# QizhiPei/FABind

Hardware: AMD Instinct MI355X
Metric: complexes/sec fwd+bwd (1500p/40l nodes), full IaBNet on the whole graph (pocket model + 4-layer complex model + distance-map head on all nodes / pairs) with the pocket-cls + pocket-centre + coord + distmap + distmap-by-coords + distill losses (BASELINE configs[2] read literally) (higher is better)
Workload: dtype bf16

## Files before the change

### fabind_amd/csrc/fused_common.h

```cpp
#pragma once
#include "common.h"

#define FE_BM 64
#define FE_PRIO(x) __builtin_amdgcn_s_setprio(x)

__device__ __forceinline__ float fe_sigmoid(float x) { return __builtin_amdgcn_rcpf(1.0f + __builtin_amdgcn_exp2f(-1.44269504f * x)); }
__device__ __forceinline__ float fe_silu(float x) { return x * fe_sigmoid(x); }

__device__ __forceinline__ uint32_t fe_hash(uint32_t x) {
    x ^= x >> 16; x *= 0x7feb352dU; x ^= x >> 15; x *= 0x846ca68bU; x ^= x >> 16;
    return x;
}
__device__ __forceinline__ float fe_keep(uint32_t seed, uint32_t e, uint32_t c, uint32_t H, uint32_t thr16, float scale) {
    const uint32_t h = fe_hash(seed + (e >> 1) * H + c);
    return (((e & 1u) ? (h >> 16) : (h & 0xffffu)) >= thr16) ? scale : 0.f;
}

__device__ __forceinline__ void unpack8(const uint4 u, float* f) {
    f[0] = __uint_as_float(u.x << 16); f[1] = __uint_as_float(u.x & 0xffff0000u);
    f[2] = __uint_as_float(u.y << 16); f[3] = __uint_as_float(u.y & 0xffff0000u);
    f[4] = __uint_as_float(u.z << 16); f[5] = __uint_as_float(u.z & 0xffff0000u);
    f[6] = __uint_as_float(u.w << 16); f[7] = __uint_as_float(u.w & 0xffff0000u);
}
__device__ __forceinline__ uint4 pack8(const float* f) {
// ... 268 lines not shown
        }
    }
    if (ne > 0) {
        if (first && head_cont) bnd_tile[c] = run;
        else if (tail_cont) bnd_tile[H + c] = run;
        else put(cur, run);
    }
    return pwr;
}

template <int H, bool WITH_RH, int SWZ>
__device__ __forceinline__ float fe_scan_runs64(const bf16_t* sX, const int* sRow, const float* sRh, int ne, bool head_cont,
                                                bool tail_cont, float* out, unsigned ld, float* bnd_tile, int c,
                                                bf16_t* out16 = nullptr, unsigned ld16 = 0, const bf16_t* sXlo = nullptr) {
    const int lane = threadIdx.x & 63;
    const int mine = sRow[lane], prev = sRow[max(lane - 1, 0)];
    const float rhl = WITH_RH ? sRh[lane] : 0.f;
    const unsigned long long m = __ballot(lane < ne && lane > 0 && mine != prev);
    const int c8 = c >> 3, c7 = c & 7;
    float v[64];
#pragma unroll
    for (int rw = 0; rw < 64; ++rw) v[rw] = bf16_to_f32(sX[rw * H + ((c8 ^ (rw & SWZ)) * 8) + c7]);
    if (sXlo) {
#pragma unroll
        for (int rw = 0; rw < 64; ++rw) v[rw] += bf16_to_f32(sXlo[rw * H + ((c8 ^ (rw & SWZ)) * 8) + c7]);
    }
    float run = 0.f, pwr = 0.f;
    int rs = 0;
    auto flush = [&](bool last) {
        if (rs == 0 && head_cont) bnd_tile[c] = run;
        else if (last && tail_cont) bnd_tile[H + c] = run;
        else {
            const unsigned node = (unsigned)__builtin_amdgcn_readlane(mine, rs);
            if (out) out[node * ld + c] = run;
            if (out16) out16[node * ld16 + c] = f32_to_bf16(run);
        }
    };
#pragma unroll
    for (int rw = 0; rw < 64; ++rw) {
        if (rw < ne) {
            if ((m >> rw) & 1ull) {
                flush(false);
                run = 0.f;
                rs = rw;
            }
            run += v[rw];
            if (WITH_RH) pwr += __builtin_bit_cast(float, __builtin_amdgcn_readlane(__builtin_bit_cast(int, rhl), rw)) * v[rw];
        }
    }
    if (ne > 0) flush(true);
    return pwr;
}

template <int BM>
__global__ void fe_boundary_fix_kernel(const int* __restrict__ row, int E, int H, const float* __restrict__ bnd, float* out,
                                       unsigned ld, bf16_t* out16 = nullptr, unsigned ld16 = 0) {
    const int t = blockIdx.x, e0 = t * BM, ne = min(BM, E - e0);
    if (ne <= 0 || e0 + ne >= E) return;
    const int r = row[e0 + ne - 1];
    if (row[e0 + ne] != r) return;
    if (row[e0] == r && e0 > 0 && row[e0 - 1] == r) return;
    for (int c = threadIdx.x; c < H; c += blockDim.x) {
        float sum = bnd[((size_t)t * 2 + 1) * H + c];
        for (int u = t + 1;; ++u) {
            const int f0 = u * BM, fn = min(BM, E - f0);
            sum += bnd[((size_t)u * 2) * H + c];
            const bool through = row[f0 + fn - 1] == r && f0 + fn < E && row[f0 + fn] == r;
            if (!through) break;
        }
        if (out) out[(unsigned)r * ld + c] = sum;
        if (out16) out16[(unsigned)r * ld16 + c] = f32_to_bf16(sum);
    }
}

__device__ __forceinline__ float fe3_row16_sum(float v) {
#define FE_DPP_ADD(ctrl_) v += __builtin_bit_cast(float, __builtin_amdgcn_update_dpp(0, __builtin_bit_cast(int, v), (ctrl_), 0xF, 0xF, true))
    FE_DPP_ADD(0xB1);
    FE_DPP_ADD(0x4E);
    FE_DPP_ADD(0x141);
    FE_DPP_ADD(0x140);
#undef FE_DPP_ADD
    return v;
}

typedef float fe_f2 __attribute__((ext_vector_type(2)));
__device__ __forceinline__ void fe3_silu_pair(const fe_f2 z, fe_f2& m, fe_f2& d) {
    const fe_f2 t = z * -1.44269504f;
    const fe_f2 o = fe_f2{__builtin_amdgcn_exp2f(t.x), __builtin_amdgcn_exp2f(t.y)} + 1.0f;
    const fe_f2 s = fe_f2{__builtin_amdgcn_rcpf(o.x), __builtin_amdgcn_rcpf(o.y)};
    m = z * s;
    d = s + (m - m * s);
}
__device__ __forceinline__ uint32_t fe3_pack(const fe_f2 v) { return pack2_bf16(v.x, v.y); }
__device__ __forceinline__ fe_f2 fe3_unpack(const uint32_t u) { return fe_f2{__uint_as_float(u << 16), __uint_as_float(u & 0xffff0000u)}; }

__device__ __forceinline__ uint4 fe3_bload16(const __amdgpu_buffer_rsrc_t rs, const unsigned voff, const unsigned soff) {
    const fe_u32x4_t v = __builtin_amdgcn_raw_buffer_load_b128(rs, (int)voff, (int)soff, 0);
    return make_uint4(v.x, v.y, v.z, v.w);
}
__device__ __forceinline__ void fe3_bstore16(const __amdgpu_buffer_rsrc_t rs, const unsigned voff, const unsigned soff, const uint4 v) {
    __builtin_amdgcn_raw_buffer_store_b128(fe_u32x4_t{v.x, v.y, v.z, v.w}, rs, (int)voff, (int)soff, 0);
}

struct FabindEdgeBwdArgs;
int fe_bwd3_launch(const FabindEdgeBwdArgs* a, int H, int bm, int n_groups, hipStream_t stream);
int fe_fwd3_launch(const float* AB, int ldab, int H, const int* row, const int* col, const float* rhohat, const float* w_r,
                   const void* W2ph, const void* W2pl, const float* b2, const void* Wcph, const void* Wcpl, const float* bc,
                   const float* w3, int E, float* agg, float* s_out, uint32_t thr16, float dscale, unsigned seed, float* bnd,
                   int xcd_aware, hipStream_t stream, void* Msave = nullptr, void* d2f = nullptr, void* z3f = nullptr);
int fe_fwd2_launch(const void* AB, int ldab, int H, const int* row, const int* col, const float* rhohat, const float* w_r,
                   const void* W2p, const float* b2, const void* Wcp, const float* bc, const float* w3, int E, float* agg,
                   float* s_out, uint32_t thr16, float dscale, unsigned seed, float* bnd, void* agg16, int xcd_aware, hipStream_t stream,
                   void* Msave = nullptr, void* d2f = nullptr, void* z3f = nullptr);
int fe_bwd4_launch(const FabindEdgeBwdArgs* a, int H, int n_groups, hipStream_t stream);
```

### fabind_amd/csrc/fused_edge.hip

```cpp
#include "common.h"
#include "fabind_hip.h"
#include "fused_common.h"

static int g_fe_xcd_aware = 1;
extern "C" void fabind_gcl_edge_fused_set_xcd_aware(int on) { g_fe_xcd_aware = on ? 1 : 0; }
static int g_fe_fwd_variant = 1;
extern "C" int fabind_gcl_edge_fused_set_variant(int v) {
    FB_REQUIRE(v == 1, "fabind_gcl_edge_fused_set_variant: 1 (row-wise / operand-swapped) is the only forward form built (variant 0 was retired in round 5)");
    g_fe_fwd_variant = v;
    return 0;
}
extern "C" int fabind_gcl_edge_fused_variant(void) { return g_fe_fwd_variant; }

static int fe_fwd_entry(const void* AB, int ldab, int H, const int* row, const int* col, const float* rhohat,
                        const float* w_r, const void* W2p, const float* b2, const void* Wcp, const float* bc,
                        const float* w3, int E, float* agg, float* s_out, float p_drop, unsigned seed,
                        float* bnd, void* agg16, void* Msave, void* d2f, void* z3f, hipStream_t stream) {
    if (E <= 0) return 0;
    FB_REQUIRE((Msave != nullptr) == (d2f != nullptr) && (Msave != nullptr) == (z3f != nullptr),
               "fabind_gcl_edge_fused_train: M, d2f and z3f come together");
    FB_REQUIRE(Msave == nullptr || g_fe_fwd_variant == 1, "fabind_gcl_edge_fused_train: the saving forward is the row-wise / operand-swapped kernel (variant 1)");
    FB_REQUIRE(bnd != nullptr, "fabind_gcl_edge_fused: bnd (ceil(E/64) x 2 x H floats of scratch) is required");
    FB_REQUIRE(p_drop >= 0.f && p_drop < 1.f, "fabind_gcl_edge_fused: p_drop in [0, 1)");
    const uint32_t thr16 = (uint32_t)(p_drop * 65536.0f + 0.5f);
    const float dscale = 1.0f / (1.0f - (float)thr16 / 65536.0f);
    FB_REQUIRE(H == 512 || H == 256 || H == 128 || H == 64, "fabind_gcl_edge_fused: H must be 64, 128, 256 or 512");
    FB_REQUIRE(ldab % 8 == 0, "fabind_gcl_edge_fused: ldab % 8");
    {
        const int rc = fe_fwd2_launch(AB, ldab, H, row, col, rhohat, w_r, W2p, b2, Wcp, bc, w3, E, agg, s_out, thr16, dscale, seed, bnd,
                                      agg16, g_fe_xcd_aware, stream, Msave, d2f, z3f);
        if (rc) return rc;
    }
    hipLaunchKernelGGL((fe_boundary_fix_kernel<FE_BM>), dim3((E + FE_BM - 1) / FE_BM), dim3(H < 256 ? H : 256), 0, stream, row, E, H,
                       bnd, agg, (unsigned)H, (bf16_t*)agg16, (unsigned)H);
    FB_CHECK_LAUNCH();
    return 0;
}

extern "C" int fabind_gcl_edge_fused(const void* AB, int ldab, int H, const int* row, const int* col, const float* rhohat,
                                     const float* w_r, const void* W2p, const float* b2, const void* Wcp, const float* bc,
                                     const float* w3, int E, float* agg, float* s_out, float p_drop, unsigned seed,
                                     float* bnd, void* agg16, hipStream_t stream) {
    return fe_fwd_entry(AB, ldab, H, row, col, rhohat, w_r, W2p, b2, Wcp, bc, w3, E, agg, s_out, p_drop, seed, bnd, agg16, nullptr, nullptr,
                        nullptr, stream);
}
extern "C" int fabind_gcl_edge_fused_train(const void* AB, int ldab, int H, const int* row, const int* col, const float* rhohat,
                                           const float* w_r, const void* W2p, const float* b2, const void* Wcp, const float* bc,
                                           const float* w3, int E, float* agg, float* s_out, float p_drop, unsigned seed,
                                           float* bnd, void* agg16, void* M, void* d2f, void* z3f, hipStream_t stream) {
    FB_REQUIRE(M != nullptr && d2f != nullptr && z3f != nullptr, "fabind_gcl_edge_fused_train: M, d2f, z3f are required");
    return fe_fwd_entry(AB, ldab, H, row, col, rhohat, w_r, W2p, b2, Wcp, bc, w3, E, agg, s_out, p_drop, seed, bnd, agg16, M, d2f, z3f, stream);
}

static int fe_x3_entry(const float* AB, int ldab, int n_rows, int H, const int* row, const int* col, const float* rhohat,
                       const float* w_r, const void* W2ph, const void* W2pl, const float* b2, const void* Wcph,
                       const void* Wcpl, const float* bc, const float* w3, int E, float* agg, float* s_out,
                       float p_drop, unsigned seed, float* bnd, void* Msave, void* d2f, void* z3f, hipStream_t stream) {
    if (E <= 0) return 0;
    FB_REQUIRE(bnd != nullptr, "fabind_gcl_edge_fused_x3: bnd (ceil(E/64) x 2 x H floats of scratch) is required");
    FB_REQUIRE(p_drop >= 0.f && p_drop < 1.f, "fabind_gcl_edge_fused_x3: p_drop in [0, 1)");
    FB_REQUIRE(H == 512 || H == 256 || H == 128 || H == 64, "fabind_gcl_edge_fused_x3: H must be 64, 128, 256 or 512");
    FB_REQUIRE(ldab % 4 == 0 && ((uintptr_t)AB & 15) == 0, "fabind_gcl_edge_fused_x3: AB must be 16-byte aligned with ldab % 4 == 0");
    FB_REQUIRE(n_rows >= 0 && (size_t)n_rows * (size_t)ldab * 4 < ((size_t)1 << 32), "fabind_gcl_edge_fused_x3: AB larger than 4 GiB (n_rows * ldab * 4 bytes): split the batch");
    const uint32_t thr16 = (uint32_t)(p_drop * 65536.0f + 0.5f);
    const float dscale = 1.0f / (1.0f - (float)thr16 / 65536.0f);
    const int rc = fe_fwd3_launch(AB, ldab, H, row, col, rhohat, w_r, W2ph, W2pl, b2, Wcph, Wcpl, bc, w3, E, agg, s_out, thr16, dscale,
                                  seed, bnd, g_fe_xcd_aware, stream, Msave, d2f, z3f);
    if (rc) return rc;
    hipLaunchKernelGGL((fe_boundary_fix_kernel<FE_BM>), dim3((E + FE_BM - 1) / FE_BM), dim3(H < 256 ? H : 256), 0, stream, row, E, H,
                       bnd, agg, (unsigned)H, (bf16_t*)nullptr, 0u);
    FB_CHECK_LAUNCH();
    return 0;
}
extern "C" int fabind_gcl_edge_fused_x3(const float* AB, int ldab, int n_rows, int H, const int* row, const int* col, const float* rhohat,
                                        const float* w_r, const void* W2ph, const void* W2pl, const float* b2, const void* Wcph,
                                        const void* Wcpl, const float* bc, const float* w3, int E, float* agg, float* s_out,
                                        float p_drop, unsigned seed, float* bnd, hipStream_t stream) {
    return fe_x3_entry(AB, ldab, n_rows, H, row, col, rhohat, w_r, W2ph, W2pl, b2, Wcph, Wcpl, bc, w3, E, agg, s_out, p_drop, seed, bnd,
                       nullptr, nullptr, nullptr, stream);
}
extern "C" int fabind_gcl_edge_fused_x3_train(const float* AB, int ldab, int n_rows, int H, const int* row, const int* col, const float* rhohat,
                                              const float* w_r, const void* W2ph, const void* W2pl, const float* b2, const void* Wcph,
                                              const void* Wcpl, const float* bc, const float* w3, int E, float* agg, float* s_out,
                                              float p_drop, unsigned seed, float* bnd, void* M, void* d2f, void* z3f, hipStream_t stream) {
    FB_REQUIRE(M != nullptr && d2f != nullptr && z3f != nullptr, "fabind_gcl_edge_fused_x3_train: M, d2f, z3f are required");
    return fe_x3_entry(AB, ldab, n_rows, H, row, col, rhohat, w_r, W2ph, W2pl, b2, Wcph, Wcpl, bc, w3, E, agg, s_out, p_drop, seed, bnd,
                       M, d2f, z3f, stream);
}

template <int H, int BM, bool DBG>
__global__ __launch_bounds__(H, (BM == 32 ? 4 : 2)) void gcl_edge_fused_bwd_kernel(const FabindEdgeBwdArgs p) {
    constexpr int TPE = H / BM;
    constexpr int CPT = BM / 8;
    constexpr int MI = BM / 16;
    extern __shared__ __attribute__((aligned(16))) unsigned char smem[];
    bf16_t* sX = (bf16_t*)smem;
    bf16_t* sY = sX + BM * H;
    int* sRow = (int*)(sY + BM * H);
    float* sDs = (float*)(sRow + BM);
    float* sRh = sDs + BM;
    const bf16_t* __restrict__ AB = (const bf16_t*)p.AB;
    const int tid = threadIdx.x, lane = tid & 63, wave = tid >> 6;
    const int fr = lane & 15, cq = lane >> 4;
    const int el = tid / TPE, cth = tid % TPE;
    const int n_tiles = (p.E + BM - 1) / BM;
    const uint32_t thr16 = (uint32_t)(p.p_drop * 65536.0f + 0.5f);
    const float dscale = 1.0f / (1.0f - (float)thr16 / 65536.0f);
    int cbase[2][2];
#pragma unroll
    for (int f0 = 0; f0 < 2; ++f0)
#pragma unroll
        for (int f2 = 0; f2 < 2; ++f2)
            cbase[f0][f2] = cq * 4 * H + (wave * 8 + (((cq & 1) ^ f2) << 2) + ((fr >> 3) ^ f0)) * 8 + (fr & 7);
#define FE_COFF(i, j, r) (cbase[(r) & 1][(j) >> 1] + ((i) * 16 + (r)) * H + ((((j) & 1) ^ ((r) >> 1)) * 16))
    long long tph[12] = {0, 0, 0, 0, 0, 0, 0, 0, 0, 0, 0, 0};
    long long tlast = 0;
#define FE_TICK(k_)                                                   \
    if constexpr (DBG) {                                              \
        const long long now_ = __builtin_readcyclecounter();         \
        tph[k_] += now_ - tlast;                                      \
        tlast = now_;                                                 \
    }
// ... 280 lines not shown

static int g_fe_bwd_bm = 64;
extern "C" int fabind_gcl_edge_fused_bwd_set_tile(int bm) {
    FB_REQUIRE(bm == 64, "fabind_gcl_edge_fused_bwd_set_tile: 64 edges per tile (the 32-edge build of the two-tile kernel was retired in round 5)");
    g_fe_bwd_bm = bm;
    return 0;
}
extern "C" int fabind_gcl_edge_fused_bwd_tile(void) { return g_fe_bwd_bm; }
static bool g_fe_bwd_variant_set = false;
static int g_fe_bwd_variant = 5;
extern "C" int fabind_gcl_edge_fused_bwd_set_variant(int v) {
    FB_REQUIRE(v == 0 || v == 5,
               "fabind_gcl_edge_fused_bwd_set_variant: 0 (two LDS tiles of 64 edges: the default for H <= 128) or 5 (row-wise, operand-swapped in-place tile + store wave: the recompute default above); variants 1-4 were knobs nobody reached and were retired in round 5");
    g_fe_bwd_variant = v;
    g_fe_bwd_variant_set = true;
    return 0;
}
extern "C" int fabind_gcl_edge_fused_bwd_variant(void) { return g_fe_bwd_variant; }
extern "C" int fabind_gcl_edge_fused_bwd_variant_for(int H) {
    return (!g_fe_bwd_variant_set && g_fe_bwd_variant == 5 && H <= 128) ? 0 : g_fe_bwd_variant;
}

extern "C" int fabind_gcl_edge_fused_bwd(const FabindEdgeBwdArgs* a_in, int H, int n_groups, hipStream_t stream) {
    FabindEdgeBwdArgs a_copy = *a_in;
    a_copy.xcd_aware = g_fe_xcd_aware;
    const FabindEdgeBwdArgs* a = &a_copy;
    if (a->E <= 0 || n_groups <= 0) return 0;
    FB_REQUIRE(H == 512 || H == 256 || H == 128 || H == 64, "fabind_gcl_edge_fused_bwd: H must be 64, 128, 256 or 512");
    FB_REQUIRE(a->ldab % 8 == 0, "fabind_gcl_edge_fused_bwd: ldab % 8");
    FB_REQUIRE(a->p_drop >= 0.f && a->p_drop < 1.f, "fabind_gcl_edge_fused_bwd: p_drop in [0, 1)");
    const int g_fe_bwd_variant = fabind_gcl_edge_fused_bwd_variant_for(H);
    if (a->d2f != nullptr || a->z3f != nullptr) {
        FB_REQUIRE(a->d2f != nullptr && a->z3f != nullptr, "fabind_gcl_edge_fused_bwd: d2f and z3f (saved by fabind_gcl_edge_fused_train) come together");
        return fe_bwd4_launch(a, H, n_groups, stream);
    }
    if (g_fe_bwd_variant == 5) return fe_bwd3_launch(a, H, 64, n_groups, stream);
    FB_REQUIRE(a->dAB16 == nullptr, "fabind_gcl_edge_fused_bwd: dAB16 (bf16 receiving-side sums) exists in variant 5 only");
    FB_REQUIRE(a->bnd != nullptr, "fabind_gcl_edge_fused_bwd: bnd (ceil(E / tile) x 2 x H floats of scratch) is required");
    const int BMr = g_fe_bwd_bm;
    const size_t lds = (size_t)2 * BMr * H * 2 + BMr * (sizeof(int) + 2 * sizeof(float));
#define FE_LAUNCH2(HH, BB)                                                                                         \
    do {                                                                                                           \
        static bool set_ = false;                                                                                  \
        if (!set_) { (void)hipFuncSetAttribute((const void*)gcl_edge_fused_bwd_kernel<HH, BB, false>, hipFuncAttributeMaxDynamicSharedMemorySize, (int)lds); set_ = true; } \
        hipLaunchKernelGGL((gcl_edge_fused_bwd_kernel<HH, BB, false>), dim3(n_groups), dim3(HH), lds, stream, *a);  \
    } while (0)
#define FE_LAUNCH(HH) FE_LAUNCH2(HH, 64)
    if (a->dbg != nullptr && H == 512) {
        static bool setd_ = false;
        if (!setd_) { (void)hipFuncSetAttribute((const void*)gcl_edge_fused_bwd_kernel<512, 64, true>, hipFuncAttributeMaxDynamicSharedMemorySize, (int)lds); }
        hipLaunchKernelGGL((gcl_edge_fused_bwd_kernel<512, 64, true>), dim3(n_groups), dim3(512), lds, stream, *a);
    } else
    if (H == 512) FE_LAUNCH(512); else if (H == 256) FE_LAUNCH(256); else if (H == 128) FE_LAUNCH(128); else FE_LAUNCH(64);
    hipLaunchKernelGGL((fe_boundary_fix_kernel<64>), dim3((a->E + 63) / 64), dim3(H < 256 ? H : 256), 0, stream, a->row, a->E, H,
                           a->bnd, a->dABrow, (unsigned)a->lddab);
#undef FE_LAUNCH
#undef FE_LAUNCH2
#undef FE_COFF
#undef FE_ROT4
#undef FE_ROT_ACC
#undef FE_ROT_D2
#undef FE_JADDR
#undef FE_LOFF
#undef FE_TICK
    FB_CHECK_LAUNCH();
    return 0;
}
```

### fabind_amd/csrc/fused_edge_bwd3.hip

```cpp
#include "common.h"
#include "fabind_hip.h"
#include "fused_common.h"
#ifndef FE3_ROT
#define FE3_ROT 0
#endif

template <int H, int SWZ>
__device__ __forceinline__ void fe3_wave_store(const bf16_t* sB, bf16_t* __restrict__ g, int e0, int ne, int lane) {
    constexpr int CH = H / 8;
    bf16_t* gt = g + (size_t)e0 * H;
    const unsigned total = (unsigned)ne * CH;
#pragma unroll 8
    for (unsigned q = lane; q < total; q += 64) {
        const unsigned rw = q / CH, ch = q % CH;
        *(uint4*)&gt[rw * H + ch * 8] = *(const uint4*)&sB[rw * H + ((ch ^ (rw & SWZ)) * 8)];
    }
}

template <int H, int SWZ>
__device__ __forceinline__ void fe3_wave_store_nt(const bf16_t* sB, bf16_t* __restrict__ g, int e0, int ne, int lane) {
    constexpr int CH = H / 8;
    const __amdgpu_buffer_rsrc_t rs = fe_rsrc(g + (size_t)e0 * H, (unsigned)ne * H * 2);
    const unsigned total = (unsigned)ne * CH;
#pragma unroll 8
// ... 352 lines not shown
                    if (ch == 0 && e < ne) (p.drh + e0)[(unsigned)e] = dot;
                }
            }
        }
        __syncthreads();
        FE_TICK(8)

        if (has_next) fetch_tables(tile + t_step);
        if (!(xf & 16)) {
            const bool head_cont = e0 > 0 && p.row[e0 - 1] == sRow[0];
            const bool tail_cont = e0 + ne < p.E && p.row[e0 + ne] == sRow[ne - 1];
            sPart[3 * H + tid] += fe_scan_rows<H, true, BM, SWZ>(sX, sRow, sRh, ne, head_cont, tail_cont, p.dAB16 ? nullptr : p.dABrow, (unsigned)p.lddab,
                                                         p.bnd + (size_t)tile * 2 * H, tid, (bf16_t*)p.dAB16, (unsigned)p.lddab16);
        }
        if (has_next) commit_tables(hb ^ 1);
        __syncthreads();
        FE_TICK(9)
    }
    if constexpr (DBG) {
        if (p.dbg && blockIdx.x == 0 && tid == 0)
            for (int k = 0; k < 12; ++k) ((long long*)p.dbg)[k] = tph[k];
    }
    __syncthreads();
    float* part = p.part + (size_t)blockIdx.x * 4 * H;
    for (int k = 0; k < 4; ++k) part[k * H + tid] = sPart[k * H + tid];
#undef FE_QOFF
#undef FE_TICK
}

static int g_fe_bwd3_exp = 0;
extern "C" void fabind_gcl_edge_fused_bwd3_set_exp(int m) { g_fe_bwd3_exp = m; }

int fe_bwd3_launch(const FabindEdgeBwdArgs* a, int H, int bm, int n_groups, hipStream_t stream) {
    FB_REQUIRE(a->d2scratch != nullptr, "fabind_gcl_edge_fused_bwd: the store-wave form needs d2scratch (n_groups x 64 x H x 2 bytes)");
    FB_REQUIRE(a->bnd != nullptr, "fabind_gcl_edge_fused_bwd: bnd (ceil(E / tile) x 2 x H floats of scratch) is required");
    FB_REQUIRE(a->lddagg % 4 == 0 && ((uintptr_t)a->dagg & 15) == 0, "fabind_gcl_edge_fused_bwd: dagg must be 16-byte aligned with lddagg % 4 == 0");
    const size_t lds = (size_t)2 * bm * H * 2 + (size_t)8 * bm * sizeof(int) + (size_t)4 * H * sizeof(float);
#define FE_LAUNCH3_(HH, BB, KK, DD)                                                                                   \
    do {                                                                                                           \
        static bool set_ = false;                                                                                  \
        if (!set_) {                                                                                               \
            const hipError_t e_ = hipFuncSetAttribute((const void*)gcl_edge_fused_bwd3_kernel<HH, BB, KK, DD>,         \
                                                      hipFuncAttributeMaxDynamicSharedMemorySize, (int)lds);       \
            if (e_ != hipSuccess) { fabind_set_error(hipGetErrorString(e_)); return (int)e_; }                     \
            set_ = true;                                                                                           \
        }                                                                                                          \
        hipLaunchKernelGGL((gcl_edge_fused_bwd3_kernel<HH, BB, KK, DD>), dim3(n_groups), dim3(HH + 64), lds, stream, *a, g_fe_bwd3_exp); \
    } while (0)
#define FE_LAUNCH3(HH, BB, DD) do { if (a->p_drop > 0.f) FE_LAUNCH3_(HH, BB, true, DD); else FE_LAUNCH3_(HH, BB, false, DD); } while (0)
    FB_REQUIRE(bm == 64, "fabind_gcl_edge_fused_bwd: the store-wave form has 64-edge tiles");
    if (a->dbg != nullptr && H == 512) FE_LAUNCH3(512, 64, true);
    else if (H == 512) FE_LAUNCH3(512, 64, false); else if (H == 256) FE_LAUNCH3(256, 64, false);
    else if (H == 128) FE_LAUNCH3(128, 64, false); else FE_LAUNCH3(64, 64, false);
    hipLaunchKernelGGL((fe_boundary_fix_kernel<64>), dim3((a->E + 63) / 64), dim3(H < 256 ? H : 256), 0, stream, a->row, a->E, H,
                       a->bnd, a->dAB16 ? nullptr : a->dABrow, (unsigned)a->lddab, (bf16_t*)a->dAB16, (unsigned)a->lddab16);
#undef FE_LAUNCH3
#undef FE_LAUNCH3_
    FB_CHECK_LAUNCH();
    return 0;
}
```

### fabind_amd/csrc/fused_edge_bwd4.hip

```cpp
#include "common.h"
#include "fabind_hip.h"
#include "fused_common.h"

#ifndef FE4_E3_DB
#define FE4_E3_DB 0
#endif
#ifndef FE4_SCAN64
#define FE4_SCAN64 0
#endif
#ifndef FE4_P5_BATCH
#define FE4_P5_BATCH 4
#endif

#ifndef FE4_NT_LOADS
#define FE4_NT_LOADS 1
#endif
#if FE4_NT_LOADS
typedef unsigned fe_u32x2_nt_t __attribute__((ext_vector_type(2)));
__device__ __forceinline__ uint2 fe4_ldq(const bf16_t* p_) { const fe_u32x2_nt_t v = __builtin_nontemporal_load((const fe_u32x2_nt_t*)p_); return make_uint2(v.x, v.y); }
#else
__device__ __forceinline__ uint2 fe4_ldq(const bf16_t* p_) { return *(const uint2*)p_; }
#endif

template <int H>
// ... 257 lines not shown
#pragma unroll
                    for (int o = 1; o < CH; o <<= 1) dot += __shfl_xor(dot, o, 64);
                }
                if (ch == 0 && e < ne) (p.drh + e0)[(unsigned)e] = dot;
            }
            }
#undef ch
        }
        __syncthreads();

        if (has_next) fetch_tables(tile + t_step);
        if (!(xf & 4)) {
            const bool head_cont = e0 > 0 && p.row[e0 - 1] == sRow[0];
            const bool tail_cont = e0 + ne < p.E && p.row[e0 + ne] == sRow[ne - 1];
#if FE4_SCAN64
            sPart[3 * H + tid] += fe_scan_runs64<H, true, SWZ>(sX, sRow, sRh, ne, head_cont, tail_cont, p.dAB16 ? nullptr : p.dABrow, (unsigned)p.lddab,
                                                              p.bnd + (size_t)tile * 2 * H, tid, (bf16_t*)p.dAB16, (unsigned)p.lddab16);
#else
            sPart[3 * H + tid] += fe_scan_rows<H, true, BM, SWZ>(sX, sRow, sRh, ne, head_cont, tail_cont, p.dAB16 ? nullptr : p.dABrow, (unsigned)p.lddab,
                                                                p.bnd + (size_t)tile * 2 * H, tid, (bf16_t*)p.dAB16, (unsigned)p.lddab16);
#endif
        }
        if (has_next) commit_tables(hb ^ 1);
        __syncthreads();
    }
    __syncthreads();
    float* part = p.part + (size_t)blockIdx.x * 4 * H;
    for (int k = 0; k < 4; ++k) part[k * H + tid] = sPart[k * H + tid];
#undef FE_QOFF
#undef FE_FOFF
#undef FE_OPAQUE
}

static int g_fe_bwd4_exp = 0;
extern "C" void fabind_gcl_edge_fused_bwd4_set_exp(int m) { g_fe_bwd4_exp = m; }

int fe_bwd4_launch(const FabindEdgeBwdArgs* a, int H, int n_groups, hipStream_t stream) {
    FB_REQUIRE(a->bnd != nullptr, "fabind_gcl_edge_fused_bwd: bnd (ceil(E / 64) x 2 x H floats of scratch) is required");
    FB_REQUIRE(a->lddagg % 4 == 0 && ((uintptr_t)a->dagg & 15) == 0, "fabind_gcl_edge_fused_bwd: dagg must be 16-byte aligned with lddagg % 4 == 0");
    const size_t lds = (size_t)FE_BM * H * 2 + (size_t)8 * FE_BM * sizeof(int) + (size_t)4 * H * sizeof(float);
#define FE_LAUNCH4(HH)                                                                                                \
    do {                                                                                                           \
        static bool set_ = false;                                                                                  \
        if (!set_) {                                                                                               \
            const hipError_t e_ = hipFuncSetAttribute((const void*)gcl_edge_fused_bwd4_kernel<HH>,                    \
                                                      hipFuncAttributeMaxDynamicSharedMemorySize, (int)lds);       \
            if (e_ != hipSuccess) { fabind_set_error(hipGetErrorString(e_)); return (int)e_; }                     \
            set_ = true;                                                                                           \
        }                                                                                                          \
        hipLaunchKernelGGL((gcl_edge_fused_bwd4_kernel<HH>), dim3(n_groups), dim3(HH), lds, stream, *a, g_fe_bwd4_exp); \
    } while (0)
    if (H == 512) FE_LAUNCH4(512); else if (H == 256) FE_LAUNCH4(256); else if (H == 128) FE_LAUNCH4(128); else FE_LAUNCH4(64);
#undef FE_LAUNCH4
    hipLaunchKernelGGL((fe_boundary_fix_kernel<64>), dim3((a->E + 63) / 64), dim3(H < 256 ? H : 256), 0, stream, a->row, a->E, H,
                       a->bnd, a->dAB16 ? nullptr : a->dABrow, (unsigned)a->lddab, (bf16_t*)a->dAB16, (unsigned)a->lddab16);
    FB_CHECK_LAUNCH();
    return 0;
}
```

### fabind_amd/csrc/gcl.hip

```cpp
#include "common.h"
#include "fabind_hip.h"

__global__ __launch_bounds__(256) void gcl_pre_kernel(const void* __restrict__ AB, int ab_dt, int ldab, int H,
                                                      const int* row, const int* col, const float* rhohat,
                                                      const float* __restrict__ w_r, void* pre, int pre_dt, int E, int act,
                                                      void* dact_out) {
    const int lane = threadIdx.x & 63;
    int e = blockIdx.x * 4 + (threadIdx.x >> 6);
    if (e >= E) return;
    const size_t a = (size_t)row[e] * ldab, b = (size_t)col[e] * ldab + H;
    const float rh = rhohat[e];
    for (int c = lane * 4; c < H; c += 256) {
        float4 va = ld4_any(AB, ab_dt, a + c), vb = ld4_any(AB, ab_dt, b + c), w = *(const float4*)(w_r + c);
        const float4 z = make_float4(va.x + vb.x + rh * w.x, va.y + vb.y + rh * w.y, va.z + vb.z + rh * w.z,
                                     va.w + vb.w + rh * w.w);
        st4_any(pre, pre_dt, (size_t)e * H + c,
                make_float4(apply_act(z.x, act), apply_act(z.y, act), apply_act(z.z, act), apply_act(z.w, act)));
        if (dact_out)
            st4_any(dact_out, pre_dt, (size_t)e * H + c,
                    make_float4(apply_dact(z.x, act), apply_dact(z.y, act), apply_dact(z.z, act), apply_dact(z.w, act)));
    }
}

#define GP_PASSES 4
// ... 109 lines not shown

template <int NSLAB, int U>
__device__ __forceinline__ void ss_accum(const void* __restrict__ Z, int z_dt, int ldz, int H, const int* eidx, int act,
                                         int lane, int e0, int e1, int estep, F8 (&acc)[NSLAB]) {
    int ee = e0;
    for (; ee + (U - 1) * estep < e1; ee += U * estep) {
        int e[U];
#pragma unroll
        for (int u = 0; u < U; ++u) e[u] = eidx ? eidx[ee + u * estep] : ee + u * estep;
#pragma unroll
        for (int s = 0; s < NSLAB; ++s) {
            const int c = s * 512 + lane * 8;
            if (c < H) {
                F8 v[U];
#pragma unroll
                for (int u = 0; u < U; ++u) v[u] = ld8_any(Z, z_dt, (size_t)e[u] * ldz + c);
#pragma unroll
                for (int u = 0; u < U; ++u)
#pragma unroll
                    for (int k = 0; k < 8; ++k) acc[s].v[k] += apply_act(v[u].v[k], act);
            }
        }
    }
    if (ee < e1) {
        int e[U];
        bool ok[U];
#pragma unroll
        for (int u = 0; u < U; ++u) {
            ok[u] = ee + u * estep < e1;
            e[u] = ok[u] ? (eidx ? eidx[ee + u * estep] : ee + u * estep) : 0;
        }
#pragma unroll
        for (int s = 0; s < NSLAB; ++s) {
            const int c = s * 512 + lane * 8;
            if (c < H) {
                F8 v[U];
#pragma unroll
                for (int u = 0; u < U; ++u) {
                    if (ok[u]) v[u] = ld8_any(Z, z_dt, (size_t)e[u] * ldz + c);
                    else
#pragma unroll
                        for (int k = 0; k < 8; ++k) v[u].v[k] = 0.f;
                }
#pragma unroll
                for (int u = 0; u < U; ++u)
#pragma unroll
                    for (int k = 0; k < 8; ++k) acc[s].v[k] += apply_act(v[u].v[k], act);
            }
        }
    }
}

template <int NSLAB>
__global__ __launch_bounds__(256) void segment_sum_kernel(const void* __restrict__ Z, int z_dt, int ldz, int H,
                                                          const int* rowptr, const int* eidx, int act, float* out,
                                                          int ldo, int n_rows, bf16_t* out16, int ldo16, int heavy_min) {
    const int lane = threadIdx.x & 63;
    const int r = blockIdx.x * 4 + (threadIdx.x >> 6);
    if (r >= n_rows) return;
    const int e0 = rowptr[r], e1 = rowptr[r + 1];
    if (e1 - e0 > heavy_min) return;
    F8 acc[NSLAB];
#pragma unroll
    for (int s = 0; s < NSLAB; ++s)
#pragma unroll
        for (int k = 0; k < 8; ++k) acc[s].v[k] = 0.f;
    ss_accum<NSLAB, 8 / NSLAB>(Z, z_dt, ldz, H, eidx, act, lane, e0, e1, 1, acc);
#pragma unroll
    for (int s = 0; s < NSLAB; ++s) {
        const int c = s * 512 + lane * 8;
        if (c < H) {
            if (out) {
                float* o = out + (size_t)r * ldo + c;
                *(float4*)o = make_float4(acc[s].v[0], acc[s].v[1], acc[s].v[2], acc[s].v[3]);
                *(float4*)(o + 4) = make_float4(acc[s].v[4], acc[s].v[5], acc[s].v[6], acc[s].v[7]);
            }
            if (out16) st8_any(out16, FB_DT_BF16, (size_t)r * ldo16 + c, acc[s]);
        }
    }
}

template <int NSLAB>
__global__ __launch_bounds__(1024) void segment_sum_heavy_kernel(const void* __restrict__ Z, int z_dt, int ldz, int H,
                                                                 const int* rowptr, const int* eidx, int act, float* out,
                                                                 int ldo, int n_rows, bf16_t* out16, int ldo16, int rpw, int heavy_min) {
    __shared__ F8 part[15][NSLAB * 64];
    __shared__ int heavy[1024];
    __shared__ int n_heavy;
    const int lane = threadIdx.x & 63, w = threadIdx.x >> 6;
    if (threadIdx.x == 0) n_heavy = 0;
    __syncthreads();
    const int rr = blockIdx.x * rpw + threadIdx.x;
    if ((int)threadIdx.x < rpw && rr < n_rows && rowptr[rr + 1] - rowptr[rr] > heavy_min) heavy[atomicAdd(&n_heavy, 1)] = rr;
    __syncthreads();
    const int nh = n_heavy;
    for (int q = 0; q < nh; ++q) {
        const int r = heavy[q];
        F8 acc[NSLAB];
#pragma unroll
        for (int s = 0; s < NSLAB; ++s)
#pragma unroll
            for (int k = 0; k < 8; ++k) acc[s].v[k] = 0.f;
        ss_accum<NSLAB, 8 / NSLAB>(Z, z_dt, ldz, H, eidx, act, lane, rowptr[r] + w, rowptr[r + 1], 16, acc);
        if (w > 0) {
#pragma unroll
            for (int s = 0; s < NSLAB; ++s) part[w - 1][s * 64 + lane] = acc[s];
        }
// ... 159 lines not shown
```

### fabind_amd/csrc/heads.hip

```cpp
#include "common.h"
#include "fabind_hip.h"

namespace {

constexpr int LOSS_THREADS = 256;
constexpr int LOSS_TERMS = 8;

__device__ __forceinline__ float agent_load(const float* p) { return __hip_atomic_load(p, __ATOMIC_RELAXED, __HIP_MEMORY_SCOPE_AGENT); }
__device__ __forceinline__ void agent_store(float* p, float v) { __hip_atomic_store(p, v, __ATOMIC_RELAXED, __HIP_MEMORY_SCOPE_AGENT); }

__device__ __forceinline__ float cls_target(const void* cls, int cls_dt, long i) {
    switch (cls_dt) {
        case 0: return ((const float*)cls)[i];
        case 1: return (float)((const long long*)cls)[i];
        case 2: return (float)((const int*)cls)[i];
        default: return (float)((const uint8_t*)cls)[i];
    }
}

__global__ __launch_bounds__(LOSS_THREADS) void loss_fwd_kernel(
    const float* __restrict__ coords, const float* __restrict__ coords_true, long n_coord, const float* __restrict__ y_pred,
    const float* __restrict__ y_by, const float* __restrict__ dis_map, long n_pair, const float* __restrict__ logits,
    const void* __restrict__ cls, int cls_dt, const uint8_t* __restrict__ mask, long n_cls, const float* __restrict__ center,
    const float* __restrict__ center_true, long n_center, float w_coord, float w_pair, float w_distill, float w_cls, float w_center,
// ... 264 lines not shown
            c[j] = j < cw ? *(const float2*)(tc + (size_t)(d.c_row0 + j0 + j) * ldtc + c2) : make_float2(0.f, 0.f);
            acc[j] = make_float2(0.f, 0.f);
        }
        for (int i = i0 + il; i < i1; i += NL) {
            const float2 p = *(const float2*)(tp + (size_t)(d.p_row0 + i) * ldtp + c2);
            const bf16_t* row = dout + (size_t)(d.pair_off + (long)i * d.C + j0) * ldo;
            uint32_t u[PB_CH];
            if (cw == PB_CH) {
#pragma unroll
                for (int j = 0; j < PB_CH; ++j) u[j] = __builtin_nontemporal_load((const uint32_t*)(row + (size_t)j * ldo) + ct);
            } else {
#pragma unroll
                for (int j = 0; j < PB_CH; ++j) u[j] = j < cw ? __builtin_nontemporal_load((const uint32_t*)(row + (size_t)j * ldo) + ct) : 0u;
            }
            float ax = 0.f, ay = 0.f;
#pragma unroll
            for (int j = 0; j < PB_CH; ++j) {
                const float dx = __uint_as_float(u[j] << 16), dy = __uint_as_float(u[j] & 0xffff0000u);
                ax += dx * c[j].x; ay += dy * c[j].y;
                acc[j].x += dx * p.x; acc[j].y += dy * p.y;
            }
            float* o = dtp + (size_t)(d.p_row0 + i) * lddp + c2;
            if (ch == 0) *(float2*)o = make_float2(ax, ay);
            else { const float2 q = *(const float2*)o; *(float2*)o = make_float2(q.x + ax, q.y + ay); }
        }
        float* po = part + ((size_t)blockIdx.x * nchunk_max + ch) * PB_CH * W;
        if (NL == 1) {
#pragma unroll
            for (int j = 0; j < PB_CH; ++j)
                if (j < cw) *(float2*)(po + j * W + c2) = acc[j];
        } else {
            __syncthreads();
#pragma unroll
            for (int j = 0; j < PB_CH; ++j)
                if (j < cw) *(float2*)(sm + ((size_t)il * PB_CH + j) * W + c2) = acc[j];
            __syncthreads();
            for (int k = threadIdx.x; k < cw * W; k += 256) {
                float v = 0.f;
                for (int l = 0; l < NL; ++l) v += sm[(size_t)l * PB_CH * W + k];
                po[k] = v;
            }
        }
    }
}
template <int W>
__global__ __launch_bounds__(256) void block_hadamard_fwd_kernel(const PairBlock* __restrict__ desc, int B, const float* __restrict__ tp,
                                                                 int ldtp, const float* __restrict__ tc, int ldtc, bf16_t* out, int ldo) {
    constexpr int CT = W / 8, RP = 256 / CT;
    const int b = pb_find(desc, B, blockIdx.x);
    const PairBlock d = desc[b];
    const int i0 = (blockIdx.x - d.tile0) * PB_TP, i1 = min(d.P, i0 + PB_TP);
    if (i0 >= d.P) return;
    const int ct = threadIdx.x % CT, rg = threadIdx.x / CT, c8 = ct * 8;
    for (int i = i0; i < i1; ++i) {
        const float4 p0 = *(const float4*)(tp + (size_t)(d.p_row0 + i) * ldtp + c8), p1 = *(const float4*)(tp + (size_t)(d.p_row0 + i) * ldtp + c8 + 4);
        bf16_t* orow = out + (size_t)(d.pair_off + (long)i * d.C) * ldo + c8;
        for (int j = rg; j < d.C; j += RP) {
            const float* c = tc + (size_t)(d.c_row0 + j) * ldtc + c8;
            const float4 q0 = *(const float4*)c, q1 = *(const float4*)(c + 4);
            typedef __attribute__((ext_vector_type(4))) unsigned int nc_u4;
            const nc_u4 v = {pack2_bf16(p0.x * q0.x, p0.y * q0.y), pack2_bf16(p0.z * q0.z, p0.w * q0.w),
                             pack2_bf16(p1.x * q1.x, p1.y * q1.y), pack2_bf16(p1.z * q1.z, p1.w * q1.w)};
            __builtin_nontemporal_store(v, (nc_u4*)(orow + (size_t)j * ldo));
        }
    }
}

__global__ __launch_bounds__(256) void block_hadamard_bwd_reduce_kernel(const PairBlock* __restrict__ desc, int B, const int* __restrict__ row_b,
                                                                        int W, int nchunk_max, const float* __restrict__ part, float* dtc,
                                                                        int lddc) {
    const int r = blockIdx.x, b = row_b[r];
    const PairBlock d = desc[b];
    const int j = r - d.c_row0, ch = j / PB_CH, jj = j % PB_CH;
    const int nt = (d.P + PB_TP - 1) / PB_TP;
    for (int c = threadIdx.x; c < W; c += 256) {
        float v = 0.f;
        for (int t = 0; t < nt; ++t) v += part[(((size_t)(d.tile0 + t) * nchunk_max + ch) * PB_CH + jj) * W + c];
        dtc[(size_t)r * lddc + c] = v;
    }
}

}

extern "C" int fabind_pair_block_tile(void) { return PB_TP; }
extern "C" int fabind_pair_block_chunk(void) { return PB_CH; }

extern "C" int fabind_pair_dist_fwd(const void* desc, int B, int n_tiles, const float* xp, const float* xc, float scale, float lo, float hi,
                                    float* y, hipStream_t stream) {
    if (B <= 0 || n_tiles <= 0) return 0;
    hipLaunchKernelGGL(pair_dist_fwd_kernel, dim3(n_tiles), dim3(256), 0, stream, (const PairBlock*)desc, B, xp, xc, scale, lo, hi, y);
    FB_CHECK_LAUNCH();
    return 0;
}
extern "C" int fabind_pair_dist_bwd(const void* desc, int B, int max_C, const float* xp, const float* xc, const float* dy, float scale,
                                    float lo, float hi, float* part, float* dxc, hipStream_t stream) {
    if (B <= 0 || max_C <= 0) return 0;
    FB_REQUIRE(part && dxc, "fabind_pair_dist_bwd: scratch [B][8][max_C][3] and the output are required");
    hipLaunchKernelGGL(pair_dist_bwd_kernel, dim3(B, 8), dim3(256), 0, stream, (const PairBlock*)desc, xp, xc, dy, scale, lo, hi, max_C, part);
    FB_CHECK_LAUNCH();
    hipLaunchKernelGGL(pair_dist_bwd_reduce_kernel, dim3(B), dim3(256), 0, stream, (const PairBlock*)desc, B, max_C, part, dxc);
    FB_CHECK_LAUNCH();
    return 0;
}
extern "C" int fabind_block_hadamard_fwd(const void* desc, int B, int n_tiles, const float* tp, int ldtp, const float* tc, int ldtc, int W,
                                         void* out, int ldo, hipStream_t stream) {
    FB_REQUIRE(W == 64 || W == 128 || W == 256 || W == 512, "fabind_block_hadamard_fwd: W in {64, 128, 256, 512}");
// ... 100 lines not shown
```

Baseline: 538.4.

## Batch boundary-fix tiles per block, cache ligand rows in hadamard, cap segment-sum occupancy

The boundary-fix kernel now handles 16 tiles per block. It finds chain-start tiles with a wavefront ballot, processes up to four chains at once, and batches the continuation loads, replacing one block per tile that mostly exits early. The pair-block Hadamard forward keeps up to 44 ligand rows in registers and prefetches the next pocket row, so the ligand features are not reloaded for every pocket row. segment_sum_kernel gets a minimum-blocks launch bound of 6, which may limit registers and cause spills.

```diff
diff --git a/fabind_amd/csrc/fused_common.h b/fabind_amd/csrc/fused_common.h
--- a/fabind_amd/csrc/fused_common.h
+++ b/fabind_amd/csrc/fused_common.h
@@ -344,26 +344,73 @@
     return pwr;
 }
 
+constexpr int FE_FIX_TILES = 16;
 template <int BM>
 __global__ void fe_boundary_fix_kernel(const int* __restrict__ row, int E, int H, const float* __restrict__ bnd, float* out,
                                        unsigned ld, bf16_t* out16 = nullptr, unsigned ld16 = 0) {
-    const int t = blockIdx.x, e0 = t * BM, ne = min(BM, E - e0);
-    if (ne <= 0 || e0 + ne >= E) return;
-    const int r = row[e0 + ne - 1];
-    if (row[e0 + ne] != r) return;
-    if (row[e0] == r && e0 > 0 && row[e0 - 1] == r) return;
-    for (int c = threadIdx.x; c < H; c += blockDim.x) {
-        float sum = bnd[((size_t)t * 2 + 1) * H + c];
-        for (int u = t + 1;; ++u) {
-            const int f0 = u * BM, fn = min(BM, E - f0);
-            sum += bnd[((size_t)u * 2) * H + c];
-            const bool through = row[f0 + fn - 1] == r && f0 + fn < E && row[f0 + fn] == r;
-            if (!through) break;
-        }
-        if (out) out[(unsigned)r * ld + c] = sum;
-        if (out16) out16[(unsigned)r * ld16 + c] = f32_to_bf16(sum);
-    }
-}
+    const int nt = (E + BM - 1) / BM, tb = blockIdx.x * FE_FIX_TILES, lane = threadIdx.x & 63;
+    bool starts = false, thru = false;
+    if (tb + lane < nt) {
+        const int e0 = (tb + lane) * BM, ne = min(BM, E - e0);
+        if (e0 + ne < E) {
+            const int r = row[e0 + ne - 1];
+            if (row[e0 + ne] == r) {
+                thru = row[e0] == r;
+                starts = lane < FE_FIX_TILES && !(thru && e0 > 0 && row[e0 - 1] == r);
+            }
+        }
+    }
+    unsigned long long st = __ballot(starts);
+    const unsigned long long th = __ballot(thru);
+    auto through = [&](int u, int r) -> bool {
+        if (u - tb < 64) return (th >> (u - tb)) & 1ull;
+        const int f0 = u * BM, fn = min(BM, E - f0);
+        return row[f0 + fn - 1] == r && f0 + fn < E && row[f0 + fn] == r;
+    };
+    while (st) {
+        int t[4];
+#pragma unroll
+        for (int i = 0; i < 4; ++i) {
+            t[i] = st ? tb + __builtin_ctzll(st) : -1;
+            st &= st - 1;
+        }
+        for (int c = threadIdx.x; c < H; c += blockDim.x) {
+            float a[4], b[4];
+#pragma unroll
+            for (int i = 0; i < 4; ++i) {
+                if (t[i] >= 0) {
+                    a[i] = bnd[((size_t)t[i] * 2 + 1) * H + c];
+                    b[i] = bnd[((size_t)(t[i] + 1) * 2) * H + c];
+                }
+            }
+#pragma unroll
+            for (int i = 0; i < 4; ++i) {
+                if (t[i] >= 0) {
+                    const int r = row[min(t[i] * BM + BM, E) - 1];
+                    float sum = a[i];
+                    sum += b[i];
+                    for (int u = t[i] + 1; through(u, r);) {
+                        int n = 1;
+                        while (n < 8 && through(u + n, r)) ++n;
+                        float v[8];
+#pragma unroll
+                        for (int k = 0; k < 8; ++k)
+                            if (k < n) v[k] = bnd[((size_t)(u + 1 + k) * 2) * H + c];
+#pragma unroll
+                        for (int k = 0; k < 8; ++k)
+                            if (k < n) sum += v[k];
+                        u += n;
+                    }
+                    if (out) out[(unsigned)r * ld + c] = sum;
+                    if (out16) out16[(unsigned)r * ld16 + c] = f32_to_bf16(sum);
+                }
+            }
+        }
+    }
+}
+template <int BM>
+inline dim3 fe_boundary_fix_grid(int E) { return dim3(((E + BM - 1) / BM + FE_FIX_TILES - 1) / FE_FIX_TILES); }
+inline dim3 fe_boundary_fix_block(int H) { return dim3(H < 256 ? (H + 63) / 64 * 64 : 256); }
 
 __device__ __forceinline__ float fe3_row16_sum(float v) {
 #define FE_DPP_ADD(ctrl_) v += __builtin_bit_cast(float, __builtin_amdgcn_update_dpp(0, __builtin_bit_cast(int, v), (ctrl_), 0xF, 0xF, true))
diff --git a/fabind_amd/csrc/fused_edge.hip b/fabind_amd/csrc/fused_edge.hip
--- a/fabind_amd/csrc/fused_edge.hip
+++ b/fabind_amd/csrc/fused_edge.hip
@@ -31,7 +31,7 @@
                                       agg16, g_fe_xcd_aware, stream, Msave, d2f, z3f);
         if (rc) return rc;
     }
-    hipLaunchKernelGGL((fe_boundary_fix_kernel<FE_BM>), dim3((E + FE_BM - 1) / FE_BM), dim3(H < 256 ? H : 256), 0, stream, row, E, H,
+    hipLaunchKernelGGL((fe_boundary_fix_kernel<FE_BM>), fe_boundary_fix_grid<FE_BM>(E), fe_boundary_fix_block(H), 0, stream, row, E, H,
                        bnd, agg, (unsigned)H, (bf16_t*)agg16, (unsigned)H);
     FB_CHECK_LAUNCH();
     return 0;
@@ -67,7 +67,7 @@
     const int rc = fe_fwd3_launch(AB, ldab, H, row, col, rhohat, w_r, W2ph, W2pl, b2, Wcph, Wcpl, bc, w3, E, agg, s_out, thr16, dscale,
                                   seed, bnd, g_fe_xcd_aware, stream, Msave, d2f, z3f);
     if (rc) return rc;
-    hipLaunchKernelGGL((fe_boundary_fix_kernel<FE_BM>), dim3((E + FE_BM - 1) / FE_BM), dim3(H < 256 ? H : 256), 0, stream, row, E, H,
+    hipLaunchKernelGGL((fe_boundary_fix_kernel<FE_BM>), fe_boundary_fix_grid<FE_BM>(E), fe_boundary_fix_block(H), 0, stream, row, E, H,
                        bnd, agg, (unsigned)H, (bf16_t*)nullptr, 0u);
     FB_CHECK_LAUNCH();
     return 0;
@@ -454,7 +454,7 @@
         hipLaunchKernelGGL((gcl_edge_fused_bwd_kernel<512, 64, true>), dim3(n_groups), dim3(512), lds, stream, *a);
     } else
     if (H == 512) FE_LAUNCH(512); else if (H == 256) FE_LAUNCH(256); else if (H == 128) FE_LAUNCH(128); else FE_LAUNCH(64);
-    hipLaunchKernelGGL((fe_boundary_fix_kernel<64>), dim3((a->E + 63) / 64), dim3(H < 256 ? H : 256), 0, stream, a->row, a->E, H,
+    hipLaunchKernelGGL((fe_boundary_fix_kernel<64>), fe_boundary_fix_grid<64>(a->E), fe_boundary_fix_block(H), 0, stream, a->row, a->E, H,
                            a->bnd, a->dABrow, (unsigned)a->lddab);
 #undef FE_LAUNCH
 #undef FE_LAUNCH2
diff --git a/fabind_amd/csrc/fused_edge_bwd3.hip b/fabind_amd/csrc/fused_edge_bwd3.hip
--- a/fabind_amd/csrc/fused_edge_bwd3.hip
+++ b/fabind_amd/csrc/fused_edge_bwd3.hip
@@ -428,7 +428,7 @@
     if (a->dbg != nullptr && H == 512) FE_LAUNCH3(512, 64, true);
     else if (H == 512) FE_LAUNCH3(512, 64, false); else if (H == 256) FE_LAUNCH3(256, 64, false);
     else if (H == 128) FE_LAUNCH3(128, 64, false); else FE_LAUNCH3(64, 64, false);
-    hipLaunchKernelGGL((fe_boundary_fix_kernel<64>), dim3((a->E + 63) / 64), dim3(H < 256 ? H : 256), 0, stream, a->row, a->E, H,
+    hipLaunchKernelGGL((fe_boundary_fix_kernel<64>), fe_boundary_fix_grid<64>(a->E), fe_boundary_fix_block(H), 0, stream, a->row, a->E, H,
                        a->bnd, a->dAB16 ? nullptr : a->dABrow, (unsigned)a->lddab, (bf16_t*)a->dAB16, (unsigned)a->lddab16);
 #undef FE_LAUNCH3
 #undef FE_LAUNCH3_
diff --git a/fabind_amd/csrc/fused_edge_bwd4.hip b/fabind_amd/csrc/fused_edge_bwd4.hip
--- a/fabind_amd/csrc/fused_edge_bwd4.hip
+++ b/fabind_amd/csrc/fused_edge_bwd4.hip
@@ -333,7 +333,7 @@
     } while (0)
     if (H == 512) FE_LAUNCH4(512); else if (H == 256) FE_LAUNCH4(256); else if (H == 128) FE_LAUNCH4(128); else FE_LAUNCH4(64);
 #undef FE_LAUNCH4
-    hipLaunchKernelGGL((fe_boundary_fix_kernel<64>), dim3((a->E + 63) / 64), dim3(H < 256 ? H : 256), 0, stream, a->row, a->E, H,
+    hipLaunchKernelGGL((fe_boundary_fix_kernel<64>), fe_boundary_fix_grid<64>(a->E), fe_boundary_fix_block(H), 0, stream, a->row, a->E, H,
                        a->bnd, a->dAB16 ? nullptr : a->dABrow, (unsigned)a->lddab, (bf16_t*)a->dAB16, (unsigned)a->lddab16);
     FB_CHECK_LAUNCH();
     return 0;
diff --git a/fabind_amd/csrc/gcl.hip b/fabind_amd/csrc/gcl.hip
--- a/fabind_amd/csrc/gcl.hip
+++ b/fabind_amd/csrc/gcl.hip
@@ -185,7 +185,7 @@
 }
 
 template <int NSLAB>
-__global__ __launch_bounds__(256) void segment_sum_kernel(const void* __restrict__ Z, int z_dt, int ldz, int H,
+__global__ __launch_bounds__(256, 6) void segment_sum_kernel(const void* __restrict__ Z, int z_dt, int ldz, int H,
                                                           const int* rowptr, const int* eidx, int act, float* out,
                                                           int ldo, int n_rows, bf16_t* out16, int ldo16, int heavy_min) {
     const int lane = threadIdx.x & 63;
diff --git a/fabind_amd/csrc/heads.hip b/fabind_amd/csrc/heads.hip
--- a/fabind_amd/csrc/heads.hip
+++ b/fabind_amd/csrc/heads.hip
@@ -340,6 +340,39 @@
     const int i0 = (blockIdx.x - d.tile0) * PB_TP, i1 = min(d.P, i0 + PB_TP);
     if (i0 >= d.P) return;
     const int ct = threadIdx.x % CT, rg = threadIdx.x / CT, c8 = ct * 8;
+    typedef __attribute__((ext_vector_type(4))) unsigned int nc_u4;
+    constexpr int NR = (44 + RP - 1) / RP;
+    if (d.C <= NR * RP) {
+        float4 q0[NR], q1[NR];
+#pragma unroll
+        for (int k = 0; k < NR; ++k) {
+            const int j = rg + k * RP;
+            const float* c = tc + (size_t)(d.c_row0 + min(j, max(d.C - 1, 0))) * ldtc + c8;
+            q0[k] = j < d.C ? *(const float4*)c : make_float4(0.f, 0.f, 0.f, 0.f);
+            q1[k] = j < d.C ? *(const float4*)(c + 4) : make_float4(0.f, 0.f, 0.f, 0.f);
+        }
+        const float* prow = tp + (size_t)(d.p_row0 + i0) * ldtp + c8;
+        float4 p0 = *(const float4*)prow, p1 = *(const float4*)(prow + 4);
+        for (int i = i0; i < i1; ++i) {
+            float4 n0 = p0, n1 = p1;
+            if (i + 1 < i1) {
+                n0 = *(const float4*)(prow + (size_t)(i + 1 - i0) * ldtp);
+                n1 = *(const float4*)(prow + (size_t)(i + 1 - i0) * ldtp + 4);
+            }
+            bf16_t* orow = out + (size_t)(d.pair_off + (long)i * d.C) * ldo + c8;
+#pragma unroll
+            for (int k = 0; k < NR; ++k) {
+                const int j = rg + k * RP;
+                if (j < d.C) {
+                    const nc_u4 v = {pack2_bf16(p0.x * q0[k].x, p0.y * q0[k].y), pack2_bf16(p0.z * q0[k].z, p0.w * q0[k].w),
+                                     pack2_bf16(p1.x * q1[k].x, p1.y * q1[k].y), pack2_bf16(p1.z * q1[k].z, p1.w * q1[k].w)};
+                    __builtin_nontemporal_store(v, (nc_u4*)(orow + (size_t)j * ldo));
+                }
+            }
+            p0 = n0; p1 = n1;
+        }
+        return;
+    }
     for (int i = i0; i < i1; ++i) {
         const float4 p0 = *(const float4*)(tp + (size_t)(d.p_row0 + i) * ldtp + c8), p1 = *(const float4*)(tp + (size_t)(d.p_row0 + i) * ldtp + c8 + 4);
         bf16_t* orow = out + (size_t)(d.pair_off + (long)i * d.C) * ldo + c8;
```

After: 544.6 (median of 6 runs). No clear change (+1.1%).
